# tjtiger86/dl-swin-gan

Hardware: AMD Instinct MI355X
Metric: cine slices/sec (fwd+bwd) at 10-iter unroll, 1/2/4/8 GPU; PSNR vs ref (higher is better)
Workload: dtype fp32

## Files before the change

### dl-swin-gan_amd/csrc/conv3d.hip

```cpp
#include "dlcs_common.h"

#include <cstdlib>
#include <type_traits>

namespace {

inline size_t ws_align(size_t n) { return (n + 255) & ~(size_t)255; }
inline bool ws_ok(const void* ws, size_t have, size_t need) { return need == 0 || (ws && have >= need); }

inline long conv_tiles(long B, long D, long H, long W) { return B * (D / 4) * ((H / 4 + 1) / 2) * ((W / 4 + 1) / 2); }
inline unsigned conv_tail_tiles(long ntile) {
    const long ntail = ntile % 256;
    return ntile > ntail && ntail > 0 && ntail * 5 <= 256 ? (unsigned)ntail : 0u;
}
inline size_t conv_tail_bytes(long ntile) { return (size_t)conv_tail_tiles(ntile) * 5 * 256 * 160 * sizeof(float); }

struct PatchRanges { int nr; long pp; };
inline PatchRanges patch_ranges(long npatch, long want) {
    const long n0 = std::max<long>(1, std::min<long>(want, npatch));
    const long pp = (npatch + n0 - 1) / n0;
    return {(int)((npatch + pp - 1) / std::max<long>(1, pp)), pp};
}
constexpr size_t kWgSlabBytes = (size_t)27 * 160 * 160 * sizeof(float);

// ... 2131 lines not shown
                  int64_t N, float* C, int64_t ldc, const float* bias, int act, float* aux_out, int64_t ldaux,
                  float alpha, const float* residual, int64_t ldr, const int32_t* row_map, dlcs_stream_t stream) {
    DLCS_CHECK_ARG(aq && ainv && bq && binv && C && M > 0 && N > 0 && K > 0 && (act == 0 || act == 1 || act == 4));
    if (K % 64 || N % 64 || ((uintptr_t)aq & 15) || ((uintptr_t)bq & 15) || M * K >= (1L << 40))
        return DLCS_ERR_UNSUPPORTED_SIZE;
    GemmF8rArgs g{};
    g.a = (const unsigned char*)aq; g.ainv = ainv; g.M = (int)M;
    g.b = (const unsigned char*)bq; g.binv = binv; g.N = (int)N; g.K = (int)K;
    g.c = C; g.ldc = ldc; g.bias = bias; g.act = act; g.alpha = alpha;
    g.res = residual; g.ldr = ldr; g.row_map = row_map; g.aux_out = aux_out; g.ldaux = ldaux;
    hipLaunchKernelGGL(gemm_f8r_kernel, dim3(cdiv(M, 64), (unsigned)(N / 64)), dim3(256), 0, (hipStream_t)stream, g);
    return dlcs_launch_status();
}

size_t dlcs_conv3d_thin_pack_f16x3_bytes(int kind) {
    return (size_t)(kind == 0 ? kThinInHalfs : kThinOutHalfs) * 2 + 256;
}

int dlcs_conv3d_thin_pack_f16x3(const float* wpacked, int64_t cout, int64_t cout_pad, int64_t cin, int64_t cin_pad,
                                int kind, void* out, dlcs_stream_t stream) {
    DLCS_CHECK_ARG(wpacked && out && (kind == 0 || kind == 1) && cout <= cout_pad && cin <= cin_pad);
    if (kind == 0 ? !(cout == 160 && cout_pad == 160 && cin >= 1 && cin <= 4)
                  : !(cin == 160 && cin_pad == 160 && cout >= 1 && cout <= 4))
        return DLCS_ERR_UNSUPPORTED_SIZE;
    if ((uintptr_t)out & 15) return DLCS_ERR_UNSUPPORTED_SIZE;
    hipStream_t st = (hipStream_t)stream;
    const int halfs = kind == 0 ? kThinInHalfs : kThinOutHalfs;
    unsigned* mx = reinterpret_cast<unsigned*>(reinterpret_cast<char*>(out) + (size_t)halfs * 2 + 16);
    if (hipMemsetAsync(mx, 0, 4, st) != hipSuccess) return dlcs_launch_status();
    const long n = 27L * cout_pad * cin_pad;
    hipLaunchKernelGGL(absmax_flat_kernel, dim3((unsigned)std::min<long>(64, (n / 4 + 255) / 256)), dim3(256), 0, st,
                       wpacked, n, mx);
    hipLaunchKernelGGL(pack_thin_f16x3_grid_kernel, dim3((unsigned)((halfs / 2 + 255) / 256)), dim3(256), 0, st,
                       wpacked, (int)cout, (int)cout_pad, (int)cin, (int)cin_pad, kind, (const unsigned*)mx, (f16*)out);
    return dlcs_launch_status();
}

int dlcs_abs_row_sum_max(const float* w, int64_t rows, int64_t row_stride, int64_t n_outer, int64_t outer_stride,
                         int64_t inner, unsigned* out, dlcs_stream_t stream) {
    DLCS_CHECK_ARG(w && out && rows > 0 && rows < (1L << 31) && n_outer > 0 && inner > 0 && n_outer * inner < (1L << 31));
    hipStream_t st = (hipStream_t)stream;
    if (hipMemsetAsync(out, 0, 4, st) != hipSuccess) return dlcs_launch_status();
// ... 125 lines not shown
    if (D % 4 || H % 4 || W % 4 || thin_ld % 4 || !al16(bigplanes) || !al16(thin) ||
        (big_is_co ? (cout_pad < 160 || cin_pad < thin_ch) : (cin_pad < 160 || cout_pad < thin_ch)))
        return DLCS_ERR_UNSUPPORTED_SIZE;
    ThinWgPArgs t{};
    t.bp = (const f16*)bigplanes; t.thin = thin; t.dw = dw_packed; t.thin_max = thin_max;
    t.rows = (long)B * D * H * W;
    t.thin_ld = (int)thin_ld; t.sgn = big_is_co ? 1 : -1; t.big_is_co = big_is_co ? 1 : 0; t.thin_ch = (int)thin_ch;
    t.cout_pad = (int)cout_pad; t.cin_pad = (int)cin_pad;
    t.B = (int)B; t.D = (int)D; t.H = (int)H; t.W = (int)W;
    if (!ws_ok(workspace, workspace_bytes, dlcs_conv3d_thin_wgrad_planes_f16x3_workspace_bytes()))
        return DLCS_ERR_WORKSPACE;
    t.part = static_cast<float*>(workspace);
    return wgrad_thin_p_launch(t, (hipStream_t)stream);
}

int dlcs_conv3d_unpack_wgrad(const float* dw_packed, float* grad, int64_t cout, int64_t cin, int64_t cout_pad,
                             int64_t cin_pad, int accumulate, dlcs_stream_t stream) {
    DLCS_CHECK_ARG(dw_packed && grad && cout > 0 && cin > 0);
    hipLaunchKernelGGL(unpack_wgrad_kernel, dim3(grid_for(cout * cin * 27)), dim3(256), 0, (hipStream_t)stream,
                       dw_packed, grad, (int)cout, (int)cin, (int)cout_pad, (int)cin_pad, accumulate);
    return dlcs_launch_status();
}

}
```

### dl-swin-gan_amd/csrc/conv3d_thin_f16x3.inc

```
typedef _Float16 f16x4_t __attribute__((ext_vector_type(4)));

DLCS_DEV void mfma32h(f32x16& acc, const f16x8_t& a, const f16x8_t& b) {
    acc = __builtin_amdgcn_mfma_f32_32x32x16_f16(a, b, acc, 0, 0, 0);
}

struct XcdWalk {
    int t, end, step;
    DLCS_DEV XcdWalk(int ntiles) {
        const int per = (ntiles + 7) >> 3, x = blockIdx.x & 7;
        t = x * per + (blockIdx.x >> 3);
        end = min(ntiles, (x + 1) * per);
        step = gridDim.x >> 3;
    }
};

DLCS_DEV f32x4_t ldz4f(const float* p, bool ok) {
    return *reinterpret_cast<const f32x4_t*>(ok ? static_cast<const void*>(p) : static_cast<const void*>(g_wg_zero_row));
}

DLCS_DEV void split_f16(float x, float s, f16& h, f16& l) {
    const float u = x * s;
    h = (f16)u;
    l = (f16)(u - (float)h);
}

constexpr int kThinInHalfs = 2 * 4 * 4 * 160 * 8;
constexpr int kThinOutHalfs = 5 * 9 * 2 * 4 * 16 * 8;

__global__ void __launch_bounds__(256) pack_thin_f16x3_grid_kernel(const float* wp, int cout, int cout_pad, int cin,
                                                                   int cin_pad, int kind, const unsigned* mx, f16* out) {
    const float s = f16x3_scale(*mx);
    const int stride = gridDim.x * 256;
    if (kind == 0) {
        for (int i = blockIdx.x * 256 + threadIdx.x; i < kThinInHalfs / 2; i += stride) {
            const int j = i & 7, co = (i >> 3) % 160, kg = (i / 1280) & 3, ks = i / 5120;
            const int tap = 8 * ks + 2 * kg + (j >> 2), ci = j & 3;
            const float v = (tap < 27 && ci < cin && co < cout) ? wp[((long)tap * cout_pad + co) * cin_pad + ci] : 0.0f;
            f16 h, l;
            split_f16(v, s, h, l);
            out[i] = h;
            out[kThinInHalfs / 2 + i] = l;
        }
        if (blockIdx.x == 0 && threadIdx.x == 0) *reinterpret_cast<float*>(out + kThinInHalfs) = s;
    } else {
        for (int i = blockIdx.x * 256 + threadIdx.x; i < kThinOutHalfs / 2; i += stride) {
            const int j = i & 7, n = (i >> 3) & 15, kg = (i >> 7) & 3, kk = (i >> 9) % 9, cc = (i >> 9) / 9;
            const int kw = n >> 2, co = n & 3, tap = 3 * kk + kw, ci = 32 * cc + 8 * kg + j;
            const float v = (kw < 3 && co < cout && ci < cin) ? wp[((long)tap * cout_pad + co) * cin_pad + ci] : 0.0f;
            f16 h, l;
            split_f16(v, s, h, l);
            const int base = (cc * 9 + kk) * 1024 + (kg * 16 + n) * 8 + j;
            out[base] = h;
// ... 645 lines not shown
```

### dl-swin-gan_amd/csrc/conv3d_thin_planes.inc

```

constexpr int kTpHY = 10, kTpHX = 6, kTpHalo = 6 * kTpHY * kTpHX;
constexpr int kTpBuf = kTpHalo * 64;
constexpr int kTpPieces = kTpHalo * 8 / 64;

__global__ void __launch_bounds__(512, 1) conv3d_thin_out_p_kernel(ConvF32Args a, const f16* xp, const f16* wimg,
                                                                   long rows) {
    __shared__ __attribute__((aligned(16))) f16 smem_tp[2 * kTpBuf + kThinOutW2];
    f16* Wl = smem_tp + 2 * kTpBuf;
    for (int i = threadIdx.x; i < kThinOutW2 / 8; i += 512) {
        const int n = i % 12, rest = i / 12;
        const int kg = rest & 3, pl = (rest >> 2) & 1, ck = rest >> 3;
        reinterpret_cast<uint4*>(Wl)[i] = reinterpret_cast<const uint4*>(wimg)[(ck * 1024 + pl * 512 + (kg * 16 + n) * 8) / 8];
    }
    const float sx = f16x3_scale(*reinterpret_cast<const unsigned*>(reinterpret_cast<const char*>(xp) + rows * 640));
    const float inv = 1.0f / (sx * *reinterpret_cast<const float*>(wimg + kThinOutHalfs));
    const int nT = a.D >> 2, nY = a.H >> 2, nX = a.W >> 2;
    const int nYX = nY * nX, nYt = (nY + 1) >> 1;
    const int lane = threadIdx.x & 63, wave = __builtin_amdgcn_readfirstlane(threadIdx.x >> 6);
    const int m = lane & 15, kg = lane >> 4;
    const int wn = m < 12 ? m : 11;
    const int bias_rows = (nYX + nX + 1) * 64;

    unsigned pk[6];
#pragma unroll
// ... 481 lines not shown
    const int co = a.big_is_co ? mm : s, ci = a.big_is_co ? s : mm;
    float* d = a.dw + ((long)tap * a.cout_pad + co) * a.cin_pad + ci;
    *d += v * inv;
}

constexpr int kTwpWG = 256;

static int wgrad_thin_p_launch(const ThinWgPArgs& a, hipStream_t st) {
    const long npatch = (long)a.B * (a.D / 4) * (a.H / 4) * (a.W / 4);
    if (npatch * 64 * 640 >= (1L << 32)) return DLCS_ERR_UNSUPPORTED_SIZE;
    const int ppr = (int)((npatch + kTwpWG - 1) / kTwpWG);
    hipLaunchKernelGGL(conv3d_wgrad_thin_p_kernel, dim3(kTwpWG), dim3(512), 0, st, a, ppr);
    hipLaunchKernelGGL(wgrad_thin_p_reduce_kernel, dim3(160 * 128 / 64), dim3(256), 0, st, a, kTwpWG);
    return dlcs_launch_status();
}
```

### dl-swin-gan_amd/dl_cs/_lib.py

```python
import ctypes
import os

import torch

_HERE = os.path.dirname(os.path.abspath(__file__))
LIB_PATH = os.environ.get("DLCS_HIP_LIB", os.path.join(_HERE, "libdlcs_hip.so"))

F32, BF16 = 0, 1
_LIB = None

_P = ctypes.c_void_p
_I64 = ctypes.c_int64
_INT = ctypes.c_int
_F = ctypes.c_float
_SZ = ctypes.c_size_t

SIGNATURES = {
    "dlcs_version": [],
    "dlcs_status_string": [_INT],
    "dlcs_sense_workspace_bytes": [_I64, _I64, _I64, _I64, _I64],
    "dlcs_sense_fwd": [_P, _P, _P, _I64, _P, _I64, _I64, _I64, _I64, _I64, _I64, _P, _SZ, _P],
    "dlcs_sense_adj": [_P, _P, _P, _I64, _P, _P, _P, _F, _I64, _I64, _I64, _I64, _I64, _I64, _P, _SZ, _P],
    "dlcs_sense_normal": [_P, _P, _P, _I64, _P, _P, _F, _F, _I64, _I64, _I64, _I64, _I64, _I64, _P, _SZ, _P],
    "dlcs_sense_cg_workspace_bytes": [_I64] * 6,
# ... 54 lines not shown
    "dlcs_conv3d_k3_wgrad_f16x3_workspace_bytes": [_I64] * 4,
    "dlcs_conv3d_k3_wgrad_f16x3": [_P, _P, _P, _I64, _I64, _I64, _I64, _P, _SZ, _P],
    "dlcs_conv3d_k3_f16x3_workspace_bytes": [_I64, _I64, _I64, _I64, _INT],
    "dlcs_conv3d_k3_f16x3": [_P, _P, _P, _P, _I64, _I64, _I64, _I64, _I64, _P, _I64, _P, _I64, _F, _INT, _INT, _P, _P, _P,
                             _P, _P, _SZ, _P],
    "dlcs_conv3d_thin_pack_f16x3_bytes": [_INT],
    "dlcs_conv3d_thin_pack_f16x3": [_P, _I64, _I64, _I64, _I64, _INT, _P, _P],
    "dlcs_absmax_f32": [_P, _I64, _P, _P],
    "dlcs_conv3d_thin_f16x3_workspace_bytes": [_I64, _I64, _I64, _I64, _INT],
    "dlcs_conv3d_thin_f16x3": [_P, _I64, _I64, _P, _P, _P, _P, _I64, _I64, _I64, _I64, _I64, _I64, _P, _I64, _P,
                               _I64, _F, _INT, _INT, _P, _P, _P, _P, _P, _SZ, _P],
    "dlcs_conv3d_thin_out_planes_f16x3": [_P, _P, _P, _P, _I64, _I64, _I64, _I64, _I64, _I64, _INT, _INT, _P],
    "dlcs_conv3d_thin_wgrad_planes_f16x3_workspace_bytes": [],
    "dlcs_conv3d_thin_wgrad_planes_f16x3": [_P, _P, _I64, _I64, _P, _INT, _P, _I64, _I64, _I64, _I64, _I64, _I64,
                                            _P, _SZ, _P],
    "dlcs_conv3d_thin_wgrad_f16x3": [_P, _I64, _I64, _P, _P, _I64, _I64, _P, _P, _I64, _I64, _P, _I64, _I64, _I64,
                                     _I64, _P],
    "dlcs_swin_pre": [_INT, _P, _P, _I64, _I64, _I64, _I64, _I64, _I64, _I64, _P],
    "dlcs_swin_pre_bwd": [_INT, _P, _P, _I64, _I64, _I64, _I64, _I64, _I64, _I64, _P],
    "dlcs_swin_post": [_INT, _P, _P, _I64, _I64, _I64, _I64, _I64, _I64, _I64, _P],
    "dlcs_swin_post_bwd": [_INT, _P, _P, _I64, _I64, _I64, _I64, _I64, _I64, _I64, _P],
    "dlcs_axpby": [_INT, _INT, _P, _P, _I64, _F, _F, _P],
    "dlcs_relu_grad": [_INT, _P, _INT, _P, _I64, _P],
    "dlcs_permute": [_INT, _INT, _P, _P, _I64, _P, _P, _INT, _P],
    "dlcs_fill_bias": [_P, _P, _I64, _I64, _I64, _P],
    "dlcs_block_layout": [_INT, _INT, _P, _P, _I64, _I64, _I64, _I64, _I64, _I64, _INT, _P],
    "dlcs_cast_multi_bf16": [_I64, _P, _P, _P, _P],
    "dlcs_kt_window_average": [_P, _P, _I64, _I64, _I64, _I64, _INT, _P],
    "dlcs_kth_largest_abs": [_P, _I64, _I64, _P, _P],
    "dlcs_cplx_mask_scale": [_P, _P, _P, _I64, _I64, _I64, _P, _INT, _P],
# ... 95 lines not shown
```

### dl-swin-gan_amd/dl_cs/models/_ops.py

```python
import ctypes

import torch

from .. import _lib
from .. import diag as _diag

F32, BF16 = _lib.F32, _lib.BF16
_I64P = ctypes.POINTER(ctypes.c_int64)


def code(t_or_dtype):
    dt = t_or_dtype.dtype if torch.is_tensor(t_or_dtype) else t_or_dtype
    return _lib.dtype_code(dt)


p = _lib.ptr
S = _lib.stream
call = _lib.call


def empty(shape, dtype, device):
    return torch.empty(shape, dtype=dtype, device=device)


# ... 465 lines not shown
    if out is None:
        out = empty((rows, out_ld), torch.float32, planes.device)
    call("dlcs_conv3d_thin_out_planes_f16x3", p(planes), p(wthin), p(bias), p(out), cout, out.shape[-1], B, D, H, W,
         int(accumulate), int(relu_out), S())
    return out


def conv3d_thin_wgrad_planes(big_planes, thin, thin_ch, thin_max, big_is_co, grid, dw_packed):
    B, D, H, W = grid
    ws, nb = _ws("dlcs_conv3d_thin_wgrad_planes_f16x3", dw_packed.device)
    call("dlcs_conv3d_thin_wgrad_planes_f16x3", p(big_planes), p(thin), thin_ch, thin.shape[-1], _word(thin_max),
         int(big_is_co), p(dw_packed), dw_packed.shape[1], dw_packed.shape[2], B, D, H, W, p(ws), nb, S())
    return dw_packed


def conv3d_wgrad(x, cin, relu_in, g, cout, grid, dw_packed, vox_per_block=16384, dbias=None):
    B, D, H, W = grid
    ws, nb = _ws("dlcs_conv3d_k3_wgrad", dw_packed.device, code(x), cin, dw_packed.shape[2], cout, dw_packed.shape[1],
             int(relu_in), dbias is not None, B, D, H, W)
    call("dlcs_conv3d_k3_wgrad", code(x), p(x), cin, x.shape[-1], dw_packed.shape[2], int(relu_in),
         p(g), cout, g.shape[-1], dw_packed.shape[1], p(dw_packed), p(dbias), B, D, H, W, vox_per_block, p(ws), nb, S())
    return dw_packed


def conv_unpack_grad(dw_packed, grad, cout, cin, accumulate=1):
    call("dlcs_conv3d_unpack_wgrad", p(dw_packed), p(grad), cout, cin, dw_packed.shape[1],
         dw_packed.shape[2], int(accumulate), S())
    return grad


# ... 33 lines not shown
```

### dl-swin-gan_amd/dl_cs/models/engine.py

```python
import ctypes
import math
import weakref


import torch

from .. import diag as _diag
from . import _ops as K
from ._window import get_window_size as get_window_size_tuple


class BlockWeights:

    NAMES = ("norm1.weight", "norm1.bias", "attn.relative_position_bias_table", "attn.qkv.weight",
             "attn.qkv.bias", "attn.proj.weight", "attn.proj.bias", "norm2.weight", "norm2.bias",
             "mlp.fc1.weight", "mlp.fc1.bias", "mlp.fc2.weight", "mlp.fc2.bias")

    LINEARS = ("attn.qkv.weight", "attn.proj.weight", "mlp.fc1.weight", "mlp.fc2.weight")

    def __init__(self, params, dtype, cast=None, hr=None):
        self.p = params
        w = cast if cast is not None else [K.cast(params[n], dtype) for n in self.LINEARS]
        self.wqkv, self.wproj, self.wfc1, self.wfc2 = w
        self.hr = None
# ... 174 lines not shown


FP32_CONV = _diag.knob("DLCS_FP32_CONV", "f32" if _diag.knob("DLCS_CONV_X6", "") == "0" else "f16x3")
if FP32_CONV not in ("f16x3", "f32"):
    raise ValueError(f"DLCS_FP32_CONV={FP32_CONV!r}: 'f16x3' (default) or 'f32'")
X6 = FP32_CONV != "f32"
H3R = _diag.knob("DLCS_H3R", "1") != "0"
_EX6 = _diag.knob("DLCS_EMBED_X6", "0")
EMBED_X6 = _EX6 in ("1", "f")
UNEMBED_X6 = _EX6 in ("1", "b")


THIN_F32 = _diag.knob("DLCS_THIN_F32", "0") == "1"
K160_F32 = _diag.knob("DLCS_K160_F32", "0") == "1"
THIN_PLANES = _diag.knob("DLCS_THIN_PLANES", "1") != "0"
FWD_PLANES_ONLY = _diag.knob("DLCS_FWD_PLANES_ONLY", "1") != "0"


_CONV_NORMS = []


def clear_norm_cache():
    del _CONV_NORMS[:]


def _conv_norm(w, C, dgrad=False):
    for t, ver, dg, nrm in _CONV_NORMS:
        if t() is w and ver == w._version and dg == dgrad:
            return nrm
    if dgrad == "patch":
# ... 184 lines not shown
            o = K.conv3d(h, C, W.fin, cin, PAD_CIN, grid, bias=P["final_layer.layers.2.conv.bias"],
                         out_dtype=torch.float32)
    else:
        hmax = None
        h = _timed_conv(b, C, W.dfe, C, C, grid, bias=P["dfe_tail.bias"], res=s, res_scale=2.0, relu_out=1)
        o = K.conv3d(h, C, W.fin, cin, PAD_CIN, grid, bias=P["final_layer.layers.2.conv.bias"],
                     out_dtype=torch.float32)
    out = K.swin_post(o, (B, E, T, Y, X), pad)
    saved = dict(u=u, s=s, b=b, pout=pout, h=h, ph=ph, stages=stages, geos=geos, shape=(B, E, T, Y, X), grid=grid,
                 pad=pad, heads=heads, cin=cin, C=C, ntok=ntok, umax=umax, hmax=hmax)
    if CAPTURE is not None:
        CAPTURE.append(dict(relu_inputs=[ss["a"] for ss in stages] + [b, h], grid=grid, C=C))
    return out, saved


def swinnet_backward(W, sv, gout, grads):
    dtype = W.dtype
    P = W.p
    grid, pad, C, cin, ntok = sv["grid"], sv["pad"], sv["C"], sv["cin"], sv["ntok"]
    dev = gout.device
    rows = grid[0] * grid[1] * grid[2] * grid[3]
    flops = _conv_flops(grid, C, C)
    go = K.swin_post_bwd(gout.contiguous(), dtype, pad, PAD_CIN)
    gout_planes = W.split and not K160_F32 and DGRAD_CAPTURE is None

    def conv_grads(x_in, cin_, g, cout, wname, bname):
        dwp = torch.zeros((27, K.pad32(cout), K.pad32(cin_)), dtype=torch.float32, device=dev)
        if cin_ == C and cout == C:
            _timed("conv_wgrad", flops, K.conv3d_wgrad, x_in, cin_, 0, g, cout, grid, dwp, dbias=grads[bname])
        else:
            K.conv3d_wgrad(x_in, cin_, 0, g, cout, grid, dwp, dbias=grads[bname])
        K.conv_unpack_grad(dwp, grads[wname], cout, cin_)

    def split_wgrad(x_planes, g_planes, wname):
        dwp = torch.zeros((27, C, C), dtype=torch.float32, device=dev)
        _timed("conv_wgrad", flops, K.conv3d_wgrad_f16x3, x_planes, g_planes, grid, dwp)
        K.conv_unpack_grad(dwp, grads[wname], C, C)

    wf = K.conv_pack(P["final_layer.layers.2.conv.weight"], dtype, 1)
    if W.split:
        pg = K.planes_alloc(rows, dev)
        if W.thin_h3:
            gomax = K.absmax(go)
            if gout_planes:
                ghm = K.zeros((1,), torch.int32, dev)
                K.planes_bound(pg, rows, m0=gomax, n0=_conv_norm(P["final_layer.layers.2.conv.weight"], C, dgrad=True))
                K.conv3d_thin_f16x3(go, cin, gomax, K.thin_pack_f16x3(wf, C, cin, 0), C, C, grid, mask=sv["h"],
                                    mask_planes=sv["ph"] if sv["h"] is None else None, out_max=K.p(ghm),
                                    out_planes=pg, planes_only=True, colsum=grads["dfe_tail.bias"])
                g_h = None
            else:
                g_h = K.conv3d_thin_f16x3(go, cin, gomax, K.thin_pack_f16x3(wf, C, cin, 0), C, C, grid, mask=sv["h"],
                                          out_max=K.planes_max(pg, rows))
            dwp = torch.zeros((27, K.pad32(cin), C), dtype=torch.float32, device=dev)
            if sv["ph"] is not None:
                K.conv3d_thin_wgrad_planes(sv["ph"], go, cin, gomax, 0, grid, dwp)
            else:
                K.conv3d_thin_wgrad_f16x3(sv["h"], C, sv["hmax"], go, cin, gomax, grid, dwp)
            K.conv_unpack_grad(dwp, grads["final_layer.layers.2.conv.weight"], cin, C)
            K.colsum(go, grads["final_layer.layers.2.conv.bias"], rows=rows, C=cin, ld=go.shape[-1])
        else:
            g_h = K.conv3d(go, cin, wf, C, C, grid, relu_in=0, mask=sv["h"])
            conv_grads(sv["h"], C, go, cin, "final_layer.layers.2.conv.weight", "final_layer.layers.2.conv.bias")
        if g_h is None:
            gp = gh_pl = pg
            ghmax = ghm
        else:
            gh_pl = None
            gp = K.split2(g_h, out=pg, have_max=W.thin_h3, colsum=grads["dfe_tail.bias"])
            ghmax = gp[rows * 640:rows * 640 + 4].view(torch.int32).clone()
        pg = K.planes_alloc(rows, dev)
        if gout_planes:
            gom = K.zeros((1,), torch.int32, dev)
            K.planes_bound(pg, rows, m0=ghmax, n0=_conv_norm(P["dfe_tail.weight"], C, dgrad=True))
            _timed("conv_dgrad", flops, K.conv3d_f16x3, gp, K.conv_pack_f16x3(P["dfe_tail.weight"], 1), grid,
# ... 102 lines not shown
            K.gemm(d_tok_t, st.emb, g_in, ntok, 64 * C, C, C, 64 * C, 64 * C, b_trans=1, res=g_out, ldr=64 * C)
        in_tok = ss["inp"].view(ntok, 64 * C)
        if K.dw_grouped_ok(ntok, [(d_tok_t, in_tok)]):
            K.gemm_dw_grouped(ntok, [(d_tok_t, in_tok, grads[pre + "emb_packed"], grads[pre + "patch_embed.proj.bias"],
                                      0)])
        else:
            K.gemm(d_tok_t, ss["inp"], grads[pre + "emb_packed"], C, 64 * C, ntok, C, 64 * C, 64 * C, a_trans=1,
                   b_trans=1, accumulate=1, splitk=max(1, min(16, ntok // 256)))
            K.colsum(d_tok, grads[pre + "patch_embed.proj.bias"])
        g_out = g_in
    g_s_t = g_out
    wsfe = K.conv_pack(P["SFE.layers.2.conv.weight"], dtype, 1)
    if pgs is not None:
        if g_s_t is not None:
            K.split2(g_s_t, out=pgs, have_max=True, colsum=grads["SFE.layers.2.conv.bias"])
        g_u = K.conv3d_thin_out_planes(pgs, K.thin_pack_f16x3(wsfe, cin, C, 1), cin, PAD_CIN, grid)
        dwp = torch.zeros((27, C, K.pad32(cin)), dtype=torch.float32, device=dev)
        K.conv3d_thin_wgrad_planes(pgs, sv["u"], cin, sv["umax"], 1, grid, dwp)
        K.conv_unpack_grad(dwp, grads["SFE.layers.2.conv.weight"], C, cin)
    elif W.thin_h3:
        g_u = K.conv3d_thin_f16x3(g_s_t, C, gsmax, K.thin_pack_f16x3(wsfe, cin, C, 1), cin, PAD_CIN, grid)
        dwp = torch.zeros((27, C, K.pad32(cin)), dtype=torch.float32, device=dev)
        K.conv3d_thin_wgrad_f16x3(sv["u"], cin, sv["umax"], g_s_t, C, gsmax, grid, dwp,
                                  colsum=grads["SFE.layers.2.conv.bias"])
        K.conv_unpack_grad(dwp, grads["SFE.layers.2.conv.weight"], C, cin)
    else:
        g_u = K.conv3d(g_s_t, C, wsfe, cin, PAD_CIN, grid)
        conv_grads(sv["u"], cin, g_s_t, C, "SFE.layers.2.conv.weight", "SFE.layers.2.conv.bias")
    return K.swin_pre_bwd(g_u, sv["shape"], pad)


def unpack_patch_grads(grads, C, nstages=1):
    for k in range(nstages):
        pre = f"rs{k}."
        K.permute(grads[pre + "emb_packed"], (C, C, 4, 4, 4), (64 * C, 1, 16 * C, 4 * C, C),
                  out=grads[pre + "patch_embed.proj.weight"], accumulate=1)
        K.permute(grads[pre + "unemb_packed"], (C, C, 4, 4, 4), (1, C, 16 * C * C, 4 * C * C, C * C),
                  out=grads[pre + "patch_unembed.proj.weight"], accumulate=1)
```

### dl-swin-gan_amd/dl_cs/models/swin3D.py

```python
import os
import weakref

import torch
from torch import nn

from . import engine
from .video_swin_transformer_mri_downsample import SwinTransformer3D
from .. import _lib

_COMPUTE_DTYPE = {"bf16": torch.bfloat16, "fp32": torch.float32}.get(
    os.environ.get("DLCS_COMPUTE_DTYPE", "fp32"), torch.float32)


def set_compute_dtype(dtype):
    global _COMPUTE_DTYPE
    assert dtype in (torch.float32, torch.bfloat16)
    _COMPUTE_DTYPE = dtype


def get_compute_dtype():
    return _COMPUTE_DTYPE


DIRECT_GRADS = False
# ... 236 lines not shown
        C = W.p["SFE.layers.2.conv.bias"].shape[0]
        direct = DIRECT_GRADS and all(
            p.grad is not None and p.grad.dtype == torch.float32 and p.grad.is_contiguous() and
            p.grad.shape == p.shape for p in W.p.values())
        if DIRECT_GRADS and GRAD_READY and not direct:
            raise RuntimeError("dl_cs: GradBuckets is active but a parameter's .grad no longer points into its "
                               "bucket (optimizer.zero_grad(set_to_none=True)?); call GradBuckets.zero() "
                               "before each backward instead")
        if direct:
            grads = {n: p.grad for n, p in W.p.items()}
        else:
            grads = {n: torch.zeros_like(p) for n, p in W.p.items()}
        for k in range(meta["nstages"]):
            grads[f"rs{k}.emb_packed"] = torch.zeros((C, 64 * C), dtype=torch.float32, device=dev)
            grads[f"rs{k}.unemb_packed"] = torch.zeros((64 * C, C), dtype=torch.float32, device=dev)
        gx = engine.swinnet_backward(W, sv, gout.to(torch.complex64), grads)
        engine.unpack_patch_grads(grads, C, meta["nstages"])
        ctx.state = None
        if direct:
            for cb in GRAD_READY:
                cb(meta["module"])
            return (gx, None) + (None,) * len(meta["names"])
        return (gx, None) + tuple(grads[n] for n in meta["names"])
```

### include/dlcs.h

```cpp
#ifndef DLCS_H
#define DLCS_H

#include <stddef.h>
#include <stdint.h>

#ifdef __cplusplus
extern "C" {
#endif

#define DLCS_VERSION 1

enum dlcs_dtype { DLCS_F32 = 0, DLCS_BF16 = 1 };

enum dlcs_status {
    DLCS_OK = 0,
    DLCS_ERR_INVALID_ARG = 100001,
    DLCS_ERR_UNSUPPORTED_SIZE = 100002,
    DLCS_ERR_WORKSPACE = 100003
};

typedef void* dlcs_stream_t;

int dlcs_version(void);
const char* dlcs_status_string(int status);
// ... 183 lines not shown
                           int64_t res_ld, float res_scale, int accumulate, int relu_out, unsigned* out_max,
                           void* out_planes, float* colsum, const void* mask_planes, void* workspace,
                           size_t workspace_bytes, dlcs_stream_t stream);
int dlcs_conv3d_thin_wgrad_f16x3(const float* in, int64_t cin, int64_t cin_ld, const unsigned* in_max,
                                 const float* g, int64_t cout, int64_t g_ld, const unsigned* g_max, float* dw_packed,
                                 int64_t cout_pad, int64_t cin_pad, float* colsum, int64_t B, int64_t D, int64_t H,
                                 int64_t W, dlcs_stream_t stream);
int dlcs_conv3d_thin_out_planes_f16x3(const void* xplanes, const void* wthin, const float* bias, float* out,
                                      int64_t cout, int64_t cout_ld, int64_t B, int64_t D, int64_t H, int64_t W,
                                      int accumulate, int relu_out, dlcs_stream_t stream);
size_t dlcs_conv3d_thin_wgrad_planes_f16x3_workspace_bytes(void);
int dlcs_conv3d_thin_wgrad_planes_f16x3(const void* bigplanes, const float* thin, int64_t thin_ch, int64_t thin_ld,
                                        const unsigned* thin_max, int big_is_co, float* dw_packed, int64_t cout_pad,
                                        int64_t cin_pad, int64_t B, int64_t D, int64_t H, int64_t W, void* workspace,
                                        size_t workspace_bytes, dlcs_stream_t stream);
int dlcs_conv3d_unpack_wgrad(const float* dw_packed, float* grad, int64_t cout, int64_t cin, int64_t cout_pad,
                             int64_t cin_pad, int accumulate, dlcs_stream_t stream);

int dlcs_swin_pre(int dtype, const void* x, void* u, int64_t B, int64_t E, int64_t T, int64_t Y, int64_t X,
                  int64_t pad, int64_t ldc, dlcs_stream_t stream);
int dlcs_swin_pre_bwd(int dtype, const void* gu, void* gx, int64_t B, int64_t E, int64_t T, int64_t Y, int64_t X,
                      int64_t pad, int64_t ldc, dlcs_stream_t stream);
int dlcs_swin_post(int dtype, const void* o, void* out, int64_t B, int64_t E, int64_t T, int64_t Y, int64_t X,
                   int64_t pad, int64_t ldc, dlcs_stream_t stream);
int dlcs_swin_post_bwd(int dtype, const void* gout, void* go, int64_t B, int64_t E, int64_t T, int64_t Y, int64_t X,
                       int64_t pad, int64_t ldc, dlcs_stream_t stream);

int dlcs_relu_grad(int g_dtype, void* g, int a_dtype, const void* a, int64_t n, dlcs_stream_t stream);
int dlcs_axpby(int x_dtype, int y_dtype, const void* x, void* y, int64_t n, float a, float b, dlcs_stream_t stream);
int dlcs_permute(int src_dtype, int dst_dtype, const void* src, void* dst, int64_t ndim,
// ... 44 lines not shown
```

Before: 4.519.

## Fuse final-layer thin conv dgrad, wgrad and bias colsums into one planes kernel

Adds a fused backward kernel for the final thin conv layer. In one pass over each patch it computes the weight gradient from the saved activation planes and the data gradient, using a tap-reversed packed weight image (new pack kind 2). It also applies the ReLU mask, writes the output gradient planes and accumulates both bias column sums, replacing three or four separate launches that each re-read the inputs. It also skips computing the first layer's input gradient when autograd does not need it. The price is a large, complex kernel with high LDS use (launch bounds of 512 threads, 1 block) and extra workspace.

Result: no change. 4.556, median of 2 (+0.8%).

```diff
diff --git a/dl-swin-gan_amd/csrc/conv3d.hip b/dl-swin-gan_amd/csrc/conv3d.hip
--- a/dl-swin-gan_amd/csrc/conv3d.hip
+++ b/dl-swin-gan_amd/csrc/conv3d.hip
@@ -2169,18 +2169,18 @@
 }
 
 size_t dlcs_conv3d_thin_pack_f16x3_bytes(int kind) {
-    return (size_t)(kind == 0 ? kThinInHalfs : kThinOutHalfs) * 2 + 256;
+    return (size_t)(kind != 1 ? kThinInHalfs : kThinOutHalfs) * 2 + 256;
 }
 
 int dlcs_conv3d_thin_pack_f16x3(const float* wpacked, int64_t cout, int64_t cout_pad, int64_t cin, int64_t cin_pad,
                                 int kind, void* out, dlcs_stream_t stream) {
-    DLCS_CHECK_ARG(wpacked && out && (kind == 0 || kind == 1) && cout <= cout_pad && cin <= cin_pad);
-    if (kind == 0 ? !(cout == 160 && cout_pad == 160 && cin >= 1 && cin <= 4)
+    DLCS_CHECK_ARG(wpacked && out && kind >= 0 && kind <= 2 && cout <= cout_pad && cin <= cin_pad);
+    if (kind != 1 ? !(cout == 160 && cout_pad == 160 && cin >= 1 && cin <= 4)
                   : !(cin == 160 && cin_pad == 160 && cout >= 1 && cout <= 4))
         return DLCS_ERR_UNSUPPORTED_SIZE;
     if ((uintptr_t)out & 15) return DLCS_ERR_UNSUPPORTED_SIZE;
     hipStream_t st = (hipStream_t)stream;
-    const int halfs = kind == 0 ? kThinInHalfs : kThinOutHalfs;
+    const int halfs = kind != 1 ? kThinInHalfs : kThinOutHalfs;
     unsigned* mx = reinterpret_cast<unsigned*>(reinterpret_cast<char*>(out) + (size_t)halfs * 2 + 16);
     if (hipMemsetAsync(mx, 0, 4, st) != hipSuccess) return dlcs_launch_status();
     const long n = 27L * cout_pad * cin_pad;
@@ -2336,6 +2336,37 @@
     return wgrad_thin_p_launch(t, (hipStream_t)stream);
 }
 
+size_t dlcs_conv3d_thin_fin_bwd_planes_f16x3_workspace_bytes(void) {
+    return ws_align((size_t)kTwpWG * 160 * 128 * sizeof(float)) + 2 * ws_align(colsum_part_bytes(kTwpWG, true));
+}
+
+int dlcs_conv3d_thin_fin_bwd_planes_f16x3(const void* xplanes, const float* g, int64_t g_ch, int64_t g_ld,
+                                          const unsigned* g_max, const void* wthin_rev, void* gx_planes,
+                                          unsigned* out_max, float* colsum, float* g_colsum, float* dw_packed,
+                                          int64_t cout_pad, int64_t cin_pad, int64_t B, int64_t D, int64_t H,
+                                          int64_t W, void* workspace, size_t workspace_bytes, dlcs_stream_t stream) {
+    DLCS_CHECK_ARG(xplanes && g && g_max && wthin_rev && gx_planes && dw_packed && B > 0 && g_ch >= 1 && g_ch <= 4 &&
+                   g_ld >= 4);
+    auto al16 = [](const void* p) { return ((uintptr_t)p & 15) == 0; };
+    if (D % 4 || H % 4 || W % 4 || g_ld % 4 || !al16(xplanes) || !al16(g) || !al16(wthin_rev) || !al16(gx_planes) ||
+        cin_pad < 160 || cout_pad < g_ch)
+        return DLCS_ERR_UNSUPPORTED_SIZE;
+    if (!ws_ok(workspace, workspace_bytes, dlcs_conv3d_thin_fin_bwd_planes_f16x3_workspace_bytes()))
+        return DLCS_ERR_WORKSPACE;
+    ThinFinBwdArgs f{};
+    ThinWgPArgs& t = f.w;
+    t.bp = (const f16*)xplanes; t.thin = g; t.dw = dw_packed; t.thin_max = g_max;
+    t.rows = (long)B * D * H * W;
+    t.thin_ld = (int)g_ld; t.sgn = -1; t.big_is_co = 0; t.thin_ch = (int)g_ch;
+    t.cout_pad = (int)cout_pad; t.cin_pad = (int)cin_pad;
+    t.B = (int)B; t.D = (int)D; t.H = (int)H; t.W = (int)W;
+    t.part = static_cast<float*>(workspace);
+    f.cpart = reinterpret_cast<float*>(static_cast<char*>(workspace) + ws_align((size_t)kTwpWG * 160 * 128 * sizeof(float)));
+    f.gpart = g_colsum ? f.cpart + ws_align(colsum_part_bytes(kTwpWG, true)) / sizeof(float) : nullptr;
+    f.wimg = (const f16*)wthin_rev; f.op = (f16*)gx_planes; f.omax = out_max;
+    return thin_fin_bwd_p_launch(f, colsum, g_colsum, (hipStream_t)stream);
+}
+
 int dlcs_conv3d_unpack_wgrad(const float* dw_packed, float* grad, int64_t cout, int64_t cin, int64_t cout_pad,
                              int64_t cin_pad, int accumulate, dlcs_stream_t stream) {
     DLCS_CHECK_ARG(dw_packed && grad && cout > 0 && cin > 0);
diff --git a/dl-swin-gan_amd/csrc/conv3d_thin_f16x3.inc b/dl-swin-gan_amd/csrc/conv3d_thin_f16x3.inc
--- a/dl-swin-gan_amd/csrc/conv3d_thin_f16x3.inc
+++ b/dl-swin-gan_amd/csrc/conv3d_thin_f16x3.inc
@@ -31,11 +31,12 @@
                                                                    int cin_pad, int kind, const unsigned* mx, f16* out) {
     const float s = f16x3_scale(*mx);
     const int stride = gridDim.x * 256;
-    if (kind == 0) {
+    if (kind != 1) {
         for (int i = blockIdx.x * 256 + threadIdx.x; i < kThinInHalfs / 2; i += stride) {
             const int j = i & 7, co = (i >> 3) % 160, kg = (i / 1280) & 3, ks = i / 5120;
             const int tap = 8 * ks + 2 * kg + (j >> 2), ci = j & 3;
-            const float v = (tap < 27 && ci < cin && co < cout) ? wp[((long)tap * cout_pad + co) * cin_pad + ci] : 0.0f;
+            const int ts = kind == 2 ? 26 - tap : tap;
+            const float v = (tap < 27 && ci < cin && co < cout) ? wp[((long)ts * cout_pad + co) * cin_pad + ci] : 0.0f;
             f16 h, l;
             split_f16(v, s, h, l);
             out[i] = h;
diff --git a/dl-swin-gan_amd/csrc/conv3d_thin_planes.inc b/dl-swin-gan_amd/csrc/conv3d_thin_planes.inc
--- a/dl-swin-gan_amd/csrc/conv3d_thin_planes.inc
+++ b/dl-swin-gan_amd/csrc/conv3d_thin_planes.inc
@@ -519,3 +519,283 @@
     hipLaunchKernelGGL(wgrad_thin_p_reduce_kernel, dim3(160 * 128 / 64), dim3(256), 0, st, a, kTwpWG);
     return dlcs_launch_status();
 }
+
+struct ThinFinBwdArgs {
+    ThinWgPArgs w;
+    const f16* wimg;
+    f16* op;
+    unsigned* omax;
+    float* cpart;
+    float* gpart;
+};
+constexpr int kTfEL = 164;
+constexpr int kTfEx = 64 * kTfEL * 2 - 4 * kTwIm;
+
+__global__ void __launch_bounds__(512, 1) conv3d_thin_fin_bwd_p_kernel(ThinFinBwdArgs fa, int ppr) {
+    __shared__ __attribute__((aligned(16))) f16 smem_tfb[2 * kTwBuf + 4 * kTwIm + kTfEx];
+    const ThinWgPArgs& a = fa.w;
+    f16* IM = smem_tfb + 2 * kTwBuf;
+    float* Es = reinterpret_cast<float*>(IM);
+    const int nT = a.D >> 2, nY = a.H >> 2, nX = a.W >> 2;
+    const int npatch = a.B * nT * nY * nX;
+    const int p0 = (int)blockIdx.x * ppr, p1 = min(npatch, p0 + ppr);
+    const int tid = threadIdx.x, lane = tid & 63, wave = __builtin_amdgcn_readfirstlane(tid >> 6);
+    const float st = f16x3_scale(*a.thin_max);
+    const float inv = 1.0f / (st * *reinterpret_cast<const float*>(fa.wimg + kThinInHalfs));
+    const float ps = f16x3_scale(*reinterpret_cast<const unsigned*>(reinterpret_cast<const char*>(fa.op) + a.rows * 640));
+    unsigned boff[5];
+#pragma unroll
+    for (int k = 0; k < 5; ++k) {
+        const int wi = 8 * k + wave, wl = wi % 10, pl = (wi / 10) & 1, un = wi / 20;
+        const int c = wl * 64 + lane;
+        const int row = c / 20, kp = c - row * 20;
+        const int kl = kp ^ (((row >> 3) & 1) << 1);
+        boff[k] = (unsigned)(((un * 32 + row) * 320 + (kl >> 2) * 64 + pl * 32 + (kl & 3) * 8) * 2);
+    }
+    const unsigned lds0 = __builtin_amdgcn_readfirstlane(lds_offset(smem_tfb));
+    auto coords = [&](int patch, int& bb, int& pt, int& py, int& px) {
+        px = patch % nX;
+        int r = patch / nX;
+        py = r % nY; r /= nY;
+        pt = r % nT;
+        bb = r / nT;
+    };
+    auto issue = [&](int patch, int buf) {
+        if (patch >= p1) return;
+        const char* sb = reinterpret_cast<const char*>(a.bp) + (long)patch * 64 * 640;
+        const unsigned dst = lds0 + (unsigned)(buf * kTwBuf * 2);
+#pragma unroll
+        for (int k = 0; k < 5; ++k) {
+            const int wi = 8 * k + wave, wl = wi % 10, pl = (wi / 10) & 1, un = wi / 20;
+            glds16_s(sb, boff[k], dst + (unsigned)((un * 2 + pl) * kTwImg * 2 + wl * 1024));
+        }
+        if (wave < 4) {
+            int bb, pt, py, px;
+            coords(patch, bb, pt, py, px);
+            const int hv = min(wave * 64 + lane, 215);
+            const int ht = hv / 36, hy = (hv / 6) % 6, hx = hv % 6;
+            const int T = min(max(pt * 4 - 1 + ht, 0), a.D - 1), Y = min(max(py * 4 - 1 + hy, 0), a.H - 1),
+                      X = min(max(px * 4 - 1 + hx, 0), a.W - 1);
+            glds16(a.thin + brow(bb, T, Y, X, nT, nY, nX) * a.thin_ld,
+                   dst + (unsigned)(kTwBigB * 2 + wave * 1024));
+        }
+    };
+    f32x4_t gs4 = (f32x4_t)0.0f;
+    const int jtap = tid >> 3, tc = tid & 7;
+    const int skd = -(jtap / 9 - 1), skh = -((jtap / 3) % 3 - 1), skw = -(jtap % 3 - 1);
+    auto build = [&](int patch, int buf) {
+        if (tid >= 216) {
+            for (int i = tid - 216; i < 4 * 32 * 5; i += 512 - 216) {
+                const int img = i / 160, r = (i / 5) % 32, c = 108 + 4 * (i % 5);
+                *reinterpret_cast<f16x4_t*>(IM + img * kTwIm + r * 128 + (c ^ (((r >> 3) & 1) << 4))) = (f16x4_t)(f16)0.0f;
+            }
+            if (tid >= 448) {
+                const int v = tid - 448;
+                const int hv = ((v >> 4) + 1) * 36 + (((v >> 2) & 3) + 1) * 6 + (v & 3) + 1;
+                const f32x4_t g = *reinterpret_cast<const f32x4_t*>(
+                    reinterpret_cast<const float*>(smem_tfb + buf * kTwBuf + kTwBigB) + hv * 4);
+#pragma unroll
+                for (int e = 0; e < 4; ++e) gs4[e] += e < a.thin_ch ? g[e] : 0.0f;
+            }
+            return;
+        }
+        int bb, pt, py, px;
+        coords(patch, bb, pt, py, px);
+        const float* TR = reinterpret_cast<const float*>(smem_tfb + buf * kTwBuf + kTwBigB);
+        const int t = tc >> 1;
+        const bool tok = (unsigned)(pt * 4 + t + skd) < (unsigned)a.D;
+#pragma unroll
+        for (int j = 0; j < 8; ++j) {
+            const int y = 2 * (tc & 1) + (j >> 2), x = j & 3;
+            const bool ok = tok && (unsigned)(py * 4 + y + skh) < (unsigned)a.H && (unsigned)(px * 4 + x + skw) < (unsigned)a.W;
+            const int hv = (t + 1 + skd) * 36 + (y + 1 + skh) * 6 + (x + 1 + skw);
+            f32x4_t v = *reinterpret_cast<const f32x4_t*>(TR + hv * 4);
+            f16x4_t h, l;
+#pragma unroll
+            for (int e = 0; e < 4; ++e) {
+                const float u = (ok && e < a.thin_ch) ? v[e] * st : 0.0f;
+                const f16 hh = (f16)u;
+                h[e] = hh;
+                l[e] = (f16)(u - (float)hh);
+            }
+            const int un = t >> 1, row = (t & 1) * 16 + y * 4 + x;
+            const int col = (jtap * 4) ^ (((row >> 3) & 1) << 4);
+            *reinterpret_cast<f16x4_t*>(IM + (un * 2 + 0) * kTwIm + row * 128 + col) = h;
+            *reinterpret_cast<f16x4_t*>(IM + (un * 2 + 1) * kTwIm + row * 128 + col) = l;
+        }
+    };
+
+    const int mh = wave & 1, nq = wave >> 1;
+    f32x4_t acc[5][2];
+#pragma unroll
+    for (int i = 0; i < 5; ++i)
+#pragma unroll
+        for (int j = 0; j < 2; ++j) acc[i][j] = (f32x4_t)0.0f;
+    const int gq = lane >> 4, q = (lane >> 2) & 3, p4 = (lane & 3) * 4, swb = gq & 1;
+    auto acol = [&](int i) { return (((mh * 5 + i) ^ swb) << 4) + p4; };
+    auto bcol = [&](int j) { return (((nq * 2 + j) ^ swb) << 4) + p4; };
+    const int grow = (8 * gq + q) * 160, trow = (8 * gq + q) * 128;
+
+    const int m = lane & 15;
+    const int nt0 = wave < 2 ? 2 * wave : wave + 2, ntn = wave < 2 ? 2 : 1;
+    f16x8_t wbh[2][4], wbl[2][4];
+#pragma unroll
+    for (int jt = 0; jt < 2; ++jt)
+#pragma unroll
+        for (int ks = 0; ks < 4; ++ks) {
+            const f16* wb = fa.wimg + ((ks * 4 + gq) * 160 + 16 * min(nt0 + jt, 9) + m) * 8;
+            wbh[jt][ks] = *reinterpret_cast<const f16x8_t*>(wb);
+            wbl[jt][ks] = *reinterpret_cast<const f16x8_t*>(wb + kThinInHalfs / 2);
+        }
+    const int arow = m * 128, asw = ((m >> 3) & 1) << 4;
+    const int wkl = tid % 20, wrg = tid / 20;
+    float cs8[8] = {0.0f, 0.0f, 0.0f, 0.0f, 0.0f, 0.0f, 0.0f, 0.0f}, vmax = 0.0f;
+
+    if (p0 < p1) issue(p0, 0);
+    asm volatile("s_waitcnt vmcnt(0)" ::: "memory");
+    __syncthreads();
+    for (int p = p0; p < p1; ++p) {
+#pragma unroll
+        for (int k = 0; k < 5; ++k) asm volatile("" : "+v"(boff[k]));
+        const int buf = (p - p0) & 1;
+        issue(p + 1, buf ^ 1);
+        build(p, buf);
+        __syncthreads();
+#pragma unroll
+        for (int un = 0; un < 2; ++un) {
+            const f16* Gh = smem_tfb + buf * kTwBuf + (un * 2) * kTwImg + grow;
+            const f16* Gl = Gh + kTwImg;
+            const f16* Th = IM + (un * 2) * kTwIm + trow;
+            const f16* Tl = Th + kTwIm;
+            f16x8_t bh[2], bl[2];
+#pragma unroll
+            for (int j = 0; j < 2; ++j) {
+                bh[j] = tr_read16h(Th + bcol(j), Th + 4 * 128 + bcol(j));
+                bl[j] = tr_read16h(Tl + bcol(j), Tl + 4 * 128 + bcol(j));
+            }
+#pragma unroll
+            for (int i = 0; i < 5; ++i) {
+                const f16x8_t gh = tr_read16h(Gh + acol(i), Gh + 4 * 160 + acol(i));
+                const f16x8_t gl = tr_read16h(Gl + acol(i), Gl + 4 * 160 + acol(i));
+#pragma unroll
+                for (int j = 0; j < 2; ++j) {
+                    mfma16h(acc[i][j], gh, bh[j]);
+                    mfma16h(acc[i][j], gh, bl[j]);
+                    mfma16h(acc[i][j], gl, bh[j]);
+                }
+            }
+        }
+        f32x4_t dacc[4][2];
+#pragma unroll
+        for (int mt = 0; mt < 4; ++mt) {
+            dacc[mt][0] = (f32x4_t)0.0f;
+            dacc[mt][1] = (f32x4_t)0.0f;
+            const unsigned rsgn = ((unsigned)(p * 4 + mt) * 0x9E3779B1u) >> 16;
+            const unsigned rowm = ((rsgn >> m) & 1) ? 0x80008000u : 0u;
+            const f16* Ah = IM + ((mt >> 1) * 2) * kTwIm + (mt & 1) * 16 * 128 + arow;
+            const f16* Al = Ah + kTwIm;
+#pragma unroll
+            for (int ks = 0; ks < 4; ++ks) {
+                const int col = (32 * ks + 8 * gq) ^ asw;
+                const f16x8_t ah = __builtin_bit_cast(
+                    f16x8_t, __builtin_bit_cast(u32x4_h3, *reinterpret_cast<const f16x8_t*>(Ah + col)) ^ rowm);
+                const f16x8_t al = __builtin_bit_cast(
+                    f16x8_t, __builtin_bit_cast(u32x4_h3, *reinterpret_cast<const f16x8_t*>(Al + col)) ^ rowm);
+#pragma unroll
+                for (int jt = 0; jt < 2; ++jt) {
+                    if (jt < ntn) {
+                        mfma16h(dacc[mt][jt], al, wbh[jt][ks]);
+                        mfma16h(dacc[mt][jt], ah, wbl[jt][ks]);
+                        mfma16h(dacc[mt][jt], ah, wbh[jt][ks]);
+                    }
+                }
+            }
+#pragma unroll
+            for (int jt = 0; jt < 2; ++jt)
+#pragma unroll
+                for (int r = 0; r < 4; ++r) dacc[mt][jt][r] *= ((rsgn >> (4 * gq + r)) & 1) ? -inv : inv;
+        }
+        asm volatile("s_waitcnt vmcnt(0)" ::: "memory");
+        __syncthreads();
+#pragma unroll
+        for (int mt = 0; mt < 4; ++mt)
+#pragma unroll
+            for (int jt = 0; jt < 2; ++jt) {
+                if (jt < ntn) {
+#pragma unroll
+                    for (int r = 0; r < 4; ++r)
+                        Es[(mt * 16 + 4 * gq + r) * kTfEL + 16 * (nt0 + jt) + m] = dacc[mt][jt][r];
+                }
+            }
+        __syncthreads();
+        if (tid < 320) {
+            const f16* Gb = smem_tfb + buf * kTwBuf;
+#pragma unroll 2
+            for (int k = 0; k < 4; ++k) {
+                const int row = wrg + 16 * k, vl = row & 31;
+                const float* ep = Es + row * kTfEL + wkl * 8;
+                f32x4_t v0 = *reinterpret_cast<const f32x4_t*>(ep);
+                f32x4_t v1 = *reinterpret_cast<const f32x4_t*>(ep + 4);
+                const f16* gp = Gb + ((row >> 5) * 2) * kTwImg + vl * 160 + ((wkl ^ (((vl >> 3) & 1) << 1)) << 3);
+                const u32x4_h3 hb = *reinterpret_cast<const u32x4_h3*>(gp);
+                const u32x4_h3 lb = *reinterpret_cast<const u32x4_h3*>(gp + kTwImg);
+#pragma unroll
+                for (int e = 0; e < 8; ++e) {
+                    const unsigned nz = ((hb[e >> 1] | lb[e >> 1]) >> (16 * (e & 1))) & 0x7fffu;
+                    if (e < 4) v0[e] = nz ? v0[e] : 0.0f;
+                    else v1[e - 4] = nz ? v1[e - 4] : 0.0f;
+                }
+                put_planes8(fa.op, (long)p * 64 + row, wkl * 8, v0, v1, ps);
+#pragma unroll
+                for (int e = 0; e < 4; ++e) {
+                    cs8[e] += v0[e];
+                    cs8[4 + e] += v1[e];
+                    vmax = fmaxf(vmax, fmaxf(fabsf(v0[e]), fabsf(v1[e])));
+                }
+            }
+        }
+        __syncthreads();
+    }
+    float* pp = a.part + (long)blockIdx.x * 160 * 128;
+#pragma unroll
+    for (int i = 0; i < 5; ++i)
+#pragma unroll
+        for (int j = 0; j < 2; ++j)
+#pragma unroll
+            for (int r = 0; r < 4; ++r)
+                pp[(16 * (mh * 5 + i) + 4 * gq + r) * 128 + 16 * (nq * 2 + j) + (lane & 15)] = acc[i][j][r];
+    if (tid < 320) {
+#pragma unroll
+        for (int e = 0; e < 8; ++e) Es[wrg * 160 + wkl * 8 + e] = cs8[e];
+    }
+    if (tid >= 448) *reinterpret_cast<f32x4_t*>(Es + 16 * 160 + (tid - 448) * 4) = gs4;
+    __syncthreads();
+    if (tid < 160) {
+        float cs = 0.0f;
+#pragma unroll
+        for (int g = 0; g < 16; ++g) cs += Es[g * 160 + tid];
+        fa.cpart[blockIdx.x * 160 + tid] = cs;
+    } else if (tid < 164 && fa.gpart) {
+        float cs = 0.0f;
+        for (int v = 0; v < 64; ++v) cs += Es[16 * 160 + v * 4 + (tid - 160)];
+        fa.gpart[blockIdx.x * 160 + (tid - 160)] = cs;
+    }
+    if (fa.omax) {
+        vmax = wave_max(vmax);
+        if (lane == 0 && vmax > 0.0f && vmax > __uint_as_float(__atomic_load_n(fa.omax, __ATOMIC_RELAXED)))
+            atomicMax(fa.omax, __float_as_uint(vmax));
+    }
+}
+
+static int thin_fin_bwd_p_launch(const ThinFinBwdArgs& fa, float* colsum, float* g_colsum, hipStream_t st) {
+    const ThinWgPArgs& a = fa.w;
+    const long npatch = (long)a.B * (a.D / 4) * (a.H / 4) * (a.W / 4);
+    if (npatch * 64 * 640 >= (1L << 32)) return DLCS_ERR_UNSUPPORTED_SIZE;
+    const int ppr = (int)((npatch + kTwpWG - 1) / kTwpWG);
+    hipLaunchKernelGGL(conv3d_thin_fin_bwd_p_kernel, dim3(kTwpWG), dim3(512), 0, st, fa, ppr);
+    hipLaunchKernelGGL(wgrad_thin_p_reduce_kernel, dim3(160 * 128 / 64), dim3(256), 0, st, a, kTwpWG);
+    if (colsum) hipLaunchKernelGGL(colsum_parts_kernel, dim3(160), dim3(256), 0, st, (const float*)fa.cpart, kTwpWG, colsum);
+    if (g_colsum)
+        hipLaunchKernelGGL(colsum_parts_kernel, dim3(a.thin_ch), dim3(256), 0, st, (const float*)fa.gpart, kTwpWG, g_colsum);
+    return dlcs_launch_status();
+}
diff --git a/dl-swin-gan_amd/dl_cs/_lib.py b/dl-swin-gan_amd/dl_cs/_lib.py
--- a/dl-swin-gan_amd/dl_cs/_lib.py
+++ b/dl-swin-gan_amd/dl_cs/_lib.py
@@ -92,6 +92,9 @@
     "dlcs_conv3d_thin_wgrad_planes_f16x3_workspace_bytes": [],
     "dlcs_conv3d_thin_wgrad_planes_f16x3": [_P, _P, _I64, _I64, _P, _INT, _P, _I64, _I64, _I64, _I64, _I64, _I64,
                                             _P, _SZ, _P],
+    "dlcs_conv3d_thin_fin_bwd_planes_f16x3_workspace_bytes": [],
+    "dlcs_conv3d_thin_fin_bwd_planes_f16x3": [_P, _P, _I64, _I64, _P, _P, _P, _P, _P, _P, _P, _I64, _I64, _I64, _I64,
+                                              _I64, _I64, _P, _SZ, _P],
     "dlcs_conv3d_thin_wgrad_f16x3": [_P, _I64, _I64, _P, _P, _I64, _I64, _P, _P, _I64, _I64, _P, _I64, _I64, _I64,
                                      _I64, _P],
     "dlcs_swin_pre": [_INT, _P, _P, _I64, _I64, _I64, _I64, _I64, _I64, _I64, _P],
diff --git a/dl-swin-gan_amd/dl_cs/models/_ops.py b/dl-swin-gan_amd/dl_cs/models/_ops.py
--- a/dl-swin-gan_amd/dl_cs/models/_ops.py
+++ b/dl-swin-gan_amd/dl_cs/models/_ops.py
@@ -503,6 +503,16 @@
     return dw_packed
 
 
+def conv3d_thin_fin_bwd_planes(x_planes, g, g_ch, g_max, wthin_rev, gx_planes, grid, dw_packed, out_max=None,
+                               colsum=None, g_colsum=None):
+    B, D, H, W = grid
+    ws, nb = _ws("dlcs_conv3d_thin_fin_bwd_planes_f16x3", dw_packed.device)
+    call("dlcs_conv3d_thin_fin_bwd_planes_f16x3", p(x_planes), p(g), g_ch, g.shape[-1], _word(g_max), p(wthin_rev),
+         p(gx_planes), _word(out_max) if out_max is not None else None, p(colsum), p(g_colsum), p(dw_packed), dw_packed.shape[1],
+         dw_packed.shape[2], B, D, H, W, p(ws), nb, S())
+    return dw_packed
+
+
 def conv3d_wgrad(x, cin, relu_in, g, cout, grid, dw_packed, vox_per_block=16384, dbias=None):
     B, D, H, W = grid
     ws, nb = _ws("dlcs_conv3d_k3_wgrad", dw_packed.device, code(x), cin, dw_packed.shape[2], cout, dw_packed.shape[1],
diff --git a/dl-swin-gan_amd/dl_cs/models/engine.py b/dl-swin-gan_amd/dl_cs/models/engine.py
--- a/dl-swin-gan_amd/dl_cs/models/engine.py
+++ b/dl-swin-gan_amd/dl_cs/models/engine.py
@@ -212,6 +212,7 @@
 THIN_F32 = _diag.knob("DLCS_THIN_F32", "0") == "1"
 K160_F32 = _diag.knob("DLCS_K160_F32", "0") == "1"
 THIN_PLANES = _diag.knob("DLCS_THIN_PLANES", "1") != "0"
+THIN_FUSED = _diag.knob("DLCS_THIN_FUSED", "1") != "0"
 FWD_PLANES_ONLY = _diag.knob("DLCS_FWD_PLANES_ONLY", "1") != "0"
 
 
@@ -426,7 +427,7 @@
     return out, saved
 
 
-def swinnet_backward(W, sv, gout, grads):
+def swinnet_backward(W, sv, gout, grads, need_input_grad=True):
     dtype = W.dtype
     P = W.p
     grid, pad, C, cin, ntok = sv["grid"], sv["pad"], sv["C"], sv["cin"], sv["ntok"]
@@ -454,9 +455,17 @@
         pg = K.planes_alloc(rows, dev)
         if W.thin_h3:
             gomax = K.absmax(go)
+            dwp = torch.zeros((27, K.pad32(cin), C), dtype=torch.float32, device=dev)
+            fused = gout_planes and THIN_FUSED and sv["ph"] is not None and sv["h"] is None
             if gout_planes:
                 ghm = K.zeros((1,), torch.int32, dev)
                 K.planes_bound(pg, rows, m0=gomax, n0=_conv_norm(P["final_layer.layers.2.conv.weight"], C, dgrad=True))
+            if fused:
+                K.conv3d_thin_fin_bwd_planes(sv["ph"], go, cin, gomax, K.thin_pack_f16x3(wf, C, cin, 2), pg, grid, dwp,
+                                             out_max=K.p(ghm), colsum=grads["dfe_tail.bias"],
+                                             g_colsum=grads["final_layer.layers.2.conv.bias"])
+                g_h = None
+            elif gout_planes:
                 K.conv3d_thin_f16x3(go, cin, gomax, K.thin_pack_f16x3(wf, C, cin, 0), C, C, grid, mask=sv["h"],
                                     mask_planes=sv["ph"] if sv["h"] is None else None, out_max=K.p(ghm),
                                     out_planes=pg, planes_only=True, colsum=grads["dfe_tail.bias"])
@@ -464,13 +473,15 @@
             else:
                 g_h = K.conv3d_thin_f16x3(go, cin, gomax, K.thin_pack_f16x3(wf, C, cin, 0), C, C, grid, mask=sv["h"],
                                           out_max=K.planes_max(pg, rows))
-            dwp = torch.zeros((27, K.pad32(cin), C), dtype=torch.float32, device=dev)
-            if sv["ph"] is not None:
+            if fused:
+                pass
+            elif sv["ph"] is not None:
                 K.conv3d_thin_wgrad_planes(sv["ph"], go, cin, gomax, 0, grid, dwp)
             else:
                 K.conv3d_thin_wgrad_f16x3(sv["h"], C, sv["hmax"], go, cin, gomax, grid, dwp)
             K.conv_unpack_grad(dwp, grads["final_layer.layers.2.conv.weight"], cin, C)
-            K.colsum(go, grads["final_layer.layers.2.conv.bias"], rows=rows, C=cin, ld=go.shape[-1])
+            if not fused:
+                K.colsum(go, grads["final_layer.layers.2.conv.bias"], rows=rows, C=cin, ld=go.shape[-1])
         else:
             g_h = K.conv3d(go, cin, wf, C, C, grid, relu_in=0, mask=sv["h"])
             conv_grads(sv["h"], C, go, cin, "final_layer.layers.2.conv.weight", "final_layer.layers.2.conv.bias")
@@ -603,20 +614,22 @@
     if pgs is not None:
         if g_s_t is not None:
             K.split2(g_s_t, out=pgs, have_max=True, colsum=grads["SFE.layers.2.conv.bias"])
-        g_u = K.conv3d_thin_out_planes(pgs, K.thin_pack_f16x3(wsfe, cin, C, 1), cin, PAD_CIN, grid)
+        g_u = (K.conv3d_thin_out_planes(pgs, K.thin_pack_f16x3(wsfe, cin, C, 1), cin, PAD_CIN, grid)
+               if need_input_grad else None)
         dwp = torch.zeros((27, C, K.pad32(cin)), dtype=torch.float32, device=dev)
         K.conv3d_thin_wgrad_planes(pgs, sv["u"], cin, sv["umax"], 1, grid, dwp)
         K.conv_unpack_grad(dwp, grads["SFE.layers.2.conv.weight"], C, cin)
     elif W.thin_h3:
-        g_u = K.conv3d_thin_f16x3(g_s_t, C, gsmax, K.thin_pack_f16x3(wsfe, cin, C, 1), cin, PAD_CIN, grid)
+        g_u = (K.conv3d_thin_f16x3(g_s_t, C, gsmax, K.thin_pack_f16x3(wsfe, cin, C, 1), cin, PAD_CIN, grid)
+               if need_input_grad else None)
         dwp = torch.zeros((27, C, K.pad32(cin)), dtype=torch.float32, device=dev)
         K.conv3d_thin_wgrad_f16x3(sv["u"], cin, sv["umax"], g_s_t, C, gsmax, grid, dwp,
                                   colsum=grads["SFE.layers.2.conv.bias"])
         K.conv_unpack_grad(dwp, grads["SFE.layers.2.conv.weight"], C, cin)
     else:
-        g_u = K.conv3d(g_s_t, C, wsfe, cin, PAD_CIN, grid)
+        g_u = K.conv3d(g_s_t, C, wsfe, cin, PAD_CIN, grid) if need_input_grad else None
         conv_grads(sv["u"], cin, g_s_t, C, "SFE.layers.2.conv.weight", "SFE.layers.2.conv.bias")
-    return K.swin_pre_bwd(g_u, sv["shape"], pad)
+    return K.swin_pre_bwd(g_u, sv["shape"], pad) if need_input_grad else None
 
 
 def unpack_patch_grads(grads, C, nstages=1):
diff --git a/dl-swin-gan_amd/dl_cs/models/swin3D.py b/dl-swin-gan_amd/dl_cs/models/swin3D.py
--- a/dl-swin-gan_amd/dl_cs/models/swin3D.py
+++ b/dl-swin-gan_amd/dl_cs/models/swin3D.py
@@ -274,7 +274,7 @@
         for k in range(meta["nstages"]):
             grads[f"rs{k}.emb_packed"] = torch.zeros((C, 64 * C), dtype=torch.float32, device=dev)
             grads[f"rs{k}.unemb_packed"] = torch.zeros((64 * C, C), dtype=torch.float32, device=dev)
-        gx = engine.swinnet_backward(W, sv, gout.to(torch.complex64), grads)
+        gx = engine.swinnet_backward(W, sv, gout.to(torch.complex64), grads, need_input_grad=ctx.needs_input_grad[0])
         engine.unpack_patch_grads(grads, C, meta["nstages"])
         ctx.state = None
         if direct:
diff --git a/include/dlcs.h b/include/dlcs.h
--- a/include/dlcs.h
+++ b/include/dlcs.h
@@ -221,6 +221,12 @@
                                         const unsigned* thin_max, int big_is_co, float* dw_packed, int64_t cout_pad,
                                         int64_t cin_pad, int64_t B, int64_t D, int64_t H, int64_t W, void* workspace,
                                         size_t workspace_bytes, dlcs_stream_t stream);
+size_t dlcs_conv3d_thin_fin_bwd_planes_f16x3_workspace_bytes(void);
+int dlcs_conv3d_thin_fin_bwd_planes_f16x3(const void* xplanes, const float* g, int64_t g_ch, int64_t g_ld,
+                                          const unsigned* g_max, const void* wthin_rev, void* gx_planes,
+                                          unsigned* out_max, float* colsum, float* g_colsum, float* dw_packed,
+                                          int64_t cout_pad, int64_t cin_pad, int64_t B, int64_t D, int64_t H,
+                                          int64_t W, void* workspace, size_t workspace_bytes, dlcs_stream_t stream);
 int dlcs_conv3d_unpack_wgrad(const float* dw_packed, float* grad, int64_t cout, int64_t cin, int64_t cout_pad,
                              int64_t cin_pad, int accumulate, dlcs_stream_t stream);
 
```
